# wjmaddox/online_gp

Hardware: AMD Instinct MI355X
Metric: streaming updates/sec (WISKI, 50^3 inducing grid) (higher is better)
Workload: dtype f32

## Files before the change

include/wiski.h:

```cpp
#ifndef WISKI_H
#define WISKI_H

#include <stdint.h>

#ifdef __cplusplus
extern "C" {
#endif

#define WISKI_OK 0
#define WISKI_E_BADARG (-1)
#define WISKI_E_LAUNCH (-2)
#define WISKI_E_WORKSPACE (-3)
#define WISKI_E_NOTCONV (-4)
#define WISKI_PENDING 1

#define WISKI_MAX_DIM 4

typedef struct wiski_grid {
  int32_t d;
  int32_t g[WISKI_MAX_DIM];
  double g0[WISKI_MAX_DIM];
  double h[WISKI_MAX_DIM];
} wiski_grid;

// ... 99 lines not shown
  int32_t guard_ok;
  double shift;
} wiski_pcg_async;
int wiski_pcg_async_f32(const wiski_grid* grid, const float* d_A_st, const float* d_tcol, float kscale, const float* d_evec, const float* d_evec2, const float* d_eval, float shift, const float* d_RHS, int32_t k, float* d_U, float* d_Z, int32_t warm, double tol, int32_t max_iter, int32_t check_every, int32_t first_check, void* d_work, int64_t work_bytes, int32_t* h_iters, double* h_relres, const int32_t* d_err, int32_t* h_err, int32_t a_sym, float* d_R, void* stream, wiski_pcg_async* handle, int32_t mode);
int wiski_pcg_async_f64(const wiski_grid* grid, const double* d_A_st, const double* d_tcol, double kscale, const double* d_evec, const double* d_evec2, const double* d_eval, double shift, const double* d_RHS, int32_t k, double* d_U, double* d_Z, int32_t warm, double tol, int32_t max_iter, int32_t check_every, int32_t first_check, void* d_work, int64_t work_bytes, int32_t* h_iters, double* h_relres, const int32_t* d_err, int32_t* h_err, int32_t a_sym, double* d_R, void* stream, wiski_pcg_async* handle, int32_t mode);
int wiski_pcg_async_free(wiski_pcg_async* handle);
int wiski_pcg_async_guard(const wiski_pcg_async* handle, const void** d_guard, int64_t* expect);
int wiski_pcg_zero_regions_f32(const wiski_grid* grid, int32_t k, int32_t max_iter, void* d_work, int32_t a_sym, void** p1, int64_t* n1_bytes, void** p2, int64_t* n2_bytes);
int wiski_pcg_zero_regions_f64(const wiski_grid* grid, int32_t k, int32_t max_iter, void* d_work, int32_t a_sym, void** p1, int64_t* n1_bytes, void** p2, int64_t* n2_bytes);
int64_t wiski_scatter_bin_bytes(const wiski_grid* grid, int64_t n, int32_t elem_size);
int wiski_scatter_stats_step_f32(const wiski_grid* grid, const float* d_x, const float* d_y, const float* d_wa, const float* d_wb, const float* d_noise, int64_t n, float* d_b, float* d_A_half, float* d_cnt, const float* d_u, float* d_res, float* d_mean_out, double* d_stats, int32_t* d_err, void* z1, int64_t n1_bytes, void* z2, int64_t n2_bytes, const void* d_guard, int64_t guard_expect, void* d_bin, int64_t bin_bytes, void* stream);
int wiski_scatter_stats_step_f64(const wiski_grid* grid, const double* d_x, const double* d_y, const double* d_wa, const double* d_wb, const double* d_noise, int64_t n, double* d_b, double* d_A_half, double* d_cnt, const double* d_u, double* d_res, double* d_mean_out, double* d_stats, int32_t* d_err, void* z1, int64_t n1_bytes, void* z2, int64_t n2_bytes, const void* d_guard, int64_t guard_expect, void* d_bin, int64_t bin_bytes, void* stream);
int wiski_gather_zero_f32(const wiski_grid* grid, const float* d_x, int64_t n, const float* d_V, int32_t k, float* d_out, int32_t* d_err, void* z1, int64_t n1_bytes, void* z2, int64_t n2_bytes, int32_t* zeroed, void* stream);
int wiski_gather_zero_f64(const wiski_grid* grid, const double* d_x, int64_t n, const double* d_V, int32_t k, double* d_out, int32_t* d_err, void* z1, int64_t n1_bytes, void* z2, int64_t n2_bytes, int32_t* zeroed, void* stream);

typedef struct wiski_stream_args_f32 {
  float* d_A_half; float* d_b; float* d_cnt; double* d_stats; int32_t* d_err;
  float* d_U; float* d_Z; float* d_R;
  const float* d_tcol; float kscale; const float* d_evec; const float* d_evec2; const float* d_eval; float shift;
  double tol; int32_t max_iter; int32_t check_every; void* d_work; int64_t work_bytes;
  void* d_bin; int64_t bin_bytes;
  const wiski_shard* shard;
  const wiski_twolevel* two_level;
  int32_t keep[3];
} wiski_stream_args_f32;
typedef struct wiski_stream_args_f64 {
  double* d_A_half; double* d_b; double* d_cnt; double* d_stats; int32_t* d_err;
  double* d_U; double* d_Z; double* d_R;
  const double* d_tcol; double kscale; const double* d_evec; const double* d_evec2; const double* d_eval; double shift;
  double tol; int32_t max_iter; int32_t check_every; void* d_work; int64_t work_bytes;
  void* d_bin; int64_t bin_bytes;
  const wiski_shard* shard;
  const wiski_twolevel* two_level;
  int32_t keep[3];
} wiski_stream_args_f64;
int wiski_stream_step_f32(const wiski_grid* grid, const wiski_stream_args_f32* args, const float* d_x, const float* d_y, const float* d_wa, const float* d_wb, const float* d_noise, int64_t q, float* d_mean_out, int32_t carry, int32_t first_check, int32_t* h_iters, double* h_relres, int32_t* h_err, void* stream, wiski_pcg_async* handle, int32_t defer, int32_t* h_resumed);
int wiski_stream_step_f64(const wiski_grid* grid, const wiski_stream_args_f64* args, const double* d_x, const double* d_y, const double* d_wa, const double* d_wb, const double* d_noise, int64_t q, double* d_mean_out, int32_t carry, int32_t first_check, int32_t* h_iters, double* h_relres, int32_t* h_err, void* stream, wiski_pcg_async* handle, int32_t defer, int32_t* h_resumed);

int wiski_scatter_stats_multi_f32(const wiski_grid* grid, const float* d_x, const float* d_y, const float* d_wa, const float* d_wb, const float* d_noise, int64_t n, int32_t nout, int64_t y_stride, int64_t w_stride, float* d_b, float* d_A_half, int64_t A_stride, float* d_cnt, const float* d_u, float* d_res, double* d_stats, int32_t* d_err, void* stream);
int wiski_scatter_stats_multi_f64(const wiski_grid* grid, const double* d_x, const double* d_y, const double* d_wa, const double* d_wb, const double* d_noise, int64_t n, int32_t nout, int64_t y_stride, int64_t w_stride, double* d_b, double* d_A_half, int64_t A_stride, double* d_cnt, const double* d_u, double* d_res, double* d_stats, int32_t* d_err, void* stream);

int wiski_scatter_stats_grad_f32(const wiski_grid* grid, const float* d_x, const float* d_y, const float* d_wa, const float* d_wb, const float* d_noise, int64_t n, float* d_b, float* d_A_half, float* d_cnt, const float* d_u, float* d_res, float* d_mean_out, double* d_stats, int32_t* d_err, void* stream);
int wiski_scatter_stats_grad_f64(const wiski_grid* grid, const double* d_x, const double* d_y, const double* d_wa, const double* d_wb, const double* d_noise, int64_t n, double* d_b, double* d_A_half, double* d_cnt, const double* d_u, double* d_res, double* d_mean_out, double* d_stats, int32_t* d_err, void* stream);

typedef struct wiski_absorb_args {
  const void* d_x; const void* d_y; const void* d_wa; const void* d_wb; const void* d_noise; int64_t n;
  void* d_b; void* d_A; int32_t half; int32_t channels; void* d_cnt; double* d_stats; int32_t* d_err;
  const void* d_u; void* d_res; void* d_mean_out;
  void* z1; int64_t n1_bytes; void* z2; int64_t n2_bytes;
  const void* d_guard; int64_t guard_expect;
  void* d_bin; int64_t bin_bytes;
  int32_t g_lo; int32_t g_hi; int32_t nout; int32_t reserved;
  int64_t y_stride; int64_t w_stride; int64_t A_stride;
} wiski_absorb_args;
int wiski_absorb_f32(const wiski_grid* grid, const wiski_absorb_args* args, void* stream);
int wiski_absorb_f64(const wiski_grid* grid, const wiski_absorb_args* args, void* stream);

int wiski_scatter_stats_robust_f32(const wiski_grid* grid, const float* d_x, const float* d_y, const float* d_wa, const float* d_wb, const float* d_noise, int64_t n, float* d_b, float* d_A_half, float* d_cnt, const float* d_u, float* d_res, float* d_mean_out, double* d_stats, int32_t* d_err, const float* d_inv_scale, float huber_c, float* d_omega_out, void* stream);
int wiski_scatter_stats_robust_f64(const wiski_grid* grid, const double* d_x, const double* d_y, const double* d_wa, const double* d_wb, const double* d_noise, int64_t n, double* d_b, double* d_A_half, double* d_cnt, const double* d_u, double* d_res, double* d_mean_out, double* d_stats, int32_t* d_err, const double* d_inv_scale, double huber_c, double* d_omega_out, void* stream);
int wiski_absorb_robust_f32(const wiski_grid* grid, const wiski_absorb_args* args, const float* d_inv_scale, float huber_c, float* d_omega_out, void* stream);
int wiski_absorb_robust_f64(const wiski_grid* grid, const wiski_absorb_args* args, const double* d_inv_scale, double huber_c, double* d_omega_out, void* stream);

typedef struct wiski_window_ring {
  void* d_x; void* d_y; void* d_wa; void* d_wb; void* d_noise;
  int64_t cap; int64_t head;
} wiski_window_ring;
int wiski_scatter_stats_window_f32(const wiski_grid* grid, const float* d_x, const float* d_y, const float* d_wa, const float* d_wb, const float* d_noise, int64_t n, const wiski_window_ring* ring, float* d_b, float* d_A_half, float* d_cnt, const float* d_u, float* d_res, float* d_mean_out, double* d_stats, int32_t* d_err, int32_t* d_void_left, void* stream);
int wiski_scatter_stats_window_f64(const wiski_grid* grid, const double* d_x, const double* d_y, const double* d_wa, const double* d_wb, const double* d_noise, int64_t n, const wiski_window_ring* ring, double* d_b, double* d_A_half, double* d_cnt, const double* d_u, double* d_res, double* d_mean_out, double* d_stats, int32_t* d_err, int32_t* d_void_left, void* stream);
int wiski_absorb_window_f32(const wiski_grid* grid, const wiski_absorb_args* args, const wiski_window_ring* ring, int32_t* d_void_left, void* stream);
int wiski_absorb_window_f64(const wiski_grid* grid, const wiski_absorb_args* args, const wiski_window_ring* ring, int32_t* d_void_left, void* stream);

int wiski_scatter_stats_interval_f32(const wiski_grid* grid, const float* d_x, const float* d_lo, const float* d_hi, const float* d_pvar, double sigma2, const float* d_wa, const float* d_wb, const float* d_noise, int64_t n, float* d_b, float* d_A_half, float* d_cnt, const float* d_u, float* d_res, float* d_mean_out, double* d_stats, int32_t* d_err, float* d_ytilde_out, float* d_omega_out, double* d_logz_out, void* stream);
int wiski_scatter_stats_interval_f64(const wiski_grid* grid, const double* d_x, const double* d_lo, const double* d_hi, const double* d_pvar, double sigma2, const double* d_wa, const double* d_wb, const double* d_noise, int64_t n, double* d_b, double* d_A_half, double* d_cnt, const double* d_u, double* d_res, double* d_mean_out, double* d_stats, int32_t* d_err, double* d_ytilde_out, double* d_omega_out, double* d_logz_out, void* stream);
int wiski_absorb_interval_f32(const wiski_grid* grid, const wiski_absorb_args* args, const float* d_lo, const float* d_hi, const float* d_pvar, double sigma2, float* d_ytilde_out, float* d_omega_out, double* d_logz_out, void* stream);
int wiski_absorb_interval_f64(const wiski_grid* grid, const wiski_absorb_args* args, const double* d_lo, const double* d_hi, const double* d_pvar, double sigma2, double* d_ytilde_out, double* d_omega_out, double* d_logz_out, void* stream);

int wiski_scatter_stats_step_sharded_f32(const wiski_grid* grid, const float* d_x, const float* d_y, const float* d_wa, const float* d_wb, const float* d_noise, int64_t n, float* d_b, float* d_A_half, float* d_cnt, const float* d_u, float* d_res, float* d_mean_out, double* d_stats, int32_t* d_err, void* z1, int64_t n1_bytes, void* z2, int64_t n2_bytes, const void* d_guard, int64_t guard_expect, int32_t g_lo, int32_t g_hi, void* stream);
int wiski_scatter_stats_step_sharded_f64(const wiski_grid* grid, const double* d_x, const double* d_y, const double* d_wa, const double* d_wb, const double* d_noise, int64_t n, double* d_b, double* d_A_half, double* d_cnt, const double* d_u, double* d_res, double* d_mean_out, double* d_stats, int32_t* d_err, void* z1, int64_t n1_bytes, void* z2, int64_t n2_bytes, const void* d_guard, int64_t guard_expect, int32_t g_lo, int32_t g_hi, void* stream);
int wiski_pcg_sharded_f32(const wiski_grid* grid, const float* d_A_st, const float* d_tcol, float kscale, const float* d_evec, const float* d_evec2, const float* d_eval, float shift, const float* d_RHS, int32_t k, float* d_U, float* d_Z, int32_t warm, double tol, int32_t max_iter, int32_t check_every, int32_t first_check, void* d_work, int64_t work_bytes, int32_t* h_iters, double* h_relres, const int32_t* d_err, int32_t* h_err, int32_t a_sym, float* d_R, void* stream, wiski_pcg_async* handle, int32_t mode, const wiski_shard* shard);
int wiski_pcg_sharded_f64(const wiski_grid* grid, const double* d_A_st, const double* d_tcol, double kscale, const double* d_evec, const double* d_evec2, const double* d_eval, double shift, const double* d_RHS, int32_t k, double* d_U, double* d_Z, int32_t warm, double tol, int32_t max_iter, int32_t check_every, int32_t first_check, void* d_work, int64_t work_bytes, int32_t* h_iters, double* h_relres, const int32_t* d_err, int32_t* h_err, int32_t a_sym, double* d_R, void* stream, wiski_pcg_async* handle, int32_t mode, const wiski_shard* shard);
int wiski_pcg_twolevel_f32(const wiski_grid* grid, const float* d_A_st, const float* d_tcol, float kscale, const float* d_evec, const float* d_evec2, const float* d_eval, float shift, const float* d_RHS, int32_t k, float* d_U, float* d_Z, int32_t warm, double tol, int32_t max_iter, int32_t check_every, int32_t first_check, void* d_work, int64_t work_bytes, int32_t* h_iters, double* h_relres, const int32_t* d_err, int32_t* h_err, int32_t a_sym, float* d_R, void* stream, wiski_pcg_async* handle, int32_t mode, const wiski_shard* shard, const wiski_twolevel* two_level);
int64_t wiski_twolevel_refresh_workspace_bytes(int32_t r);
int wiski_twolevel_refresh_f32(const wiski_grid* grid, const float* d_x, int64_t n, const float* d_scale, const double* d_V, int32_t kw, const int32_t* d_S, int32_t r, const double* d_lam_unit, double kscale, double gscale, double* d_G, void* d_work, int64_t work_bytes, float* d_N, const uint64_t* d_sticky, int32_t* d_bad, void* stream);
int wiski_precond_apply_f32(const wiski_grid* grid, const float* d_evec, const float* d_evec2, const float* d_eval, float kscale, float shift, const float* d_r, float* d_w0, float* d_w1, float* d_y, float* d_t, double* d_rho, const wiski_twolevel* two_level, void* stream);
int wiski_precond_apply_keep_f32(const wiski_grid* grid, const float* d_evec, const float* d_evec2, const float* d_eval, float kscale, float shift, const float* d_r, float* d_w0, float* d_w1, float* d_y, float* d_t, double* d_rho, const wiski_twolevel* two_level, const int32_t* keep, void* stream);
int wiski_precond_keep_ok(const wiski_grid* grid, const int32_t* keep, int32_t with_two_level);
int wiski_precond_apply_cols_f32(const wiski_grid* grid, const float* d_evec, const float* d_evec2, const float* d_eval, float kscale, float shift, const float* d_r, int32_t k, float* d_w0, float* d_w1, float* d_y, float* d_t, double* d_rho, const wiski_twolevel* two_level, void* stream);

int wiski_gemm_f32(int32_t ta, int32_t tb, int32_t M, int32_t N, int32_t K, float alpha, const float* d_A, int32_t lda, const float* d_B, int32_t ldb, float beta, float* d_C, int32_t ldc, void* stream);
int wiski_gemm_f64(int32_t ta, int32_t tb, int32_t M, int32_t N, int32_t K, double alpha, const double* d_A, int32_t lda, const double* d_B, int32_t ldb, double beta, double* d_C, int32_t ldc, void* stream);
int wiski_potrf_f32(int32_t n, float* d_A, int32_t lda, int32_t* d_info, void* stream);
int wiski_potrf_f64(int32_t n, double* d_A, int32_t lda, int32_t* d_info, void* stream);
int wiski_potrf_inverse_f32(int32_t n, float* d_A, int32_t lda, float* d_X, int32_t ldx, int32_t* d_info, void* stream);
int wiski_potrf_inverse_f64(int32_t n, double* d_A, int32_t lda, double* d_X, int32_t ldx, int32_t* d_info, void* stream);
int wiski_trsm_f32(int32_t trans, int32_t n, int32_t nrhs, const float* d_L, int32_t ldl, float* d_B, int32_t ldb, void* stream);
int wiski_trsm_f64(int32_t trans, int32_t n, int32_t nrhs, const double* d_L, int32_t ldl, double* d_B, int32_t ldb, void* stream);
int wiski_logdiag_f32(int32_t n, const float* d_A, int32_t lda, double* d_out, void* stream);
int wiski_logdiag_f64(int32_t n, const double* d_A, int32_t lda, double* d_out, void* stream);

int wiski_dense_factor_f32(const wiski_grid* grid, const float* d_A_half, const float* d_evec, const float* d_eval, float kscale, float* d_work, int64_t work_elems, float* d_chol, float* d_M, double* d_logdiag, int32_t* d_info, void* stream);
int wiski_dense_factor_f64(const wiski_grid* grid, const double* d_A_half, const double* d_evec, const double* d_eval, double kscale, double* d_work, int64_t work_elems, double* d_chol, double* d_M, double* d_logdiag, int32_t* d_info, void* stream);

int64_t wiski_root_update_workspace_elems(int32_t m, int32_t r, int32_t q);
int wiski_root_update_f32(int32_t m, int32_t r, int32_t q, float* d_L, int32_t ldl, float* d_R, int32_t ldr, const float* d_V, int32_t ldv, float* d_ws, int64_t ws_elems, void* stream);
int wiski_root_update_f64(int32_t m, int32_t r, int32_t q, double* d_L, int32_t ldl, double* d_R, int32_t ldr, const double* d_V, int32_t ldv, double* d_ws, int64_t ws_elems, void* stream);

int wiski_basis_project_f32(const wiski_grid* grid, const float* d_x, int64_t n, const double* d_V, int32_t kmax, const int32_t* d_S, int32_t r, const float* d_scale, const double* d_colscale, const double* d_tcol, double* d_F, int64_t ldf, double* d_prior, int32_t* d_err, void* stream);
int wiski_basis_project_f64(const wiski_grid* grid, const double* d_x, int64_t n, const double* d_V, int32_t kmax, const int32_t* d_S, int32_t r, const double* d_scale, const double* d_colscale, const double* d_tcol, double* d_F, int64_t ldf, double* d_prior, int32_t* d_err, void* stream);
int wiski_basis_project_vjp_f32(const wiski_grid* grid, const float* d_x, int64_t n, const double* d_V, int32_t kmax, const int32_t* d_S, int32_t r, const float* d_scale, const double* d_colscale, const double* d_tcol, const double* d_GF, int64_t ldg, const double* d_Gprior, float* d_gx, void* stream);
int wiski_basis_project_vjp_f64(const wiski_grid* grid, const double* d_x, int64_t n, const double* d_V, int32_t kmax, const int32_t* d_S, int32_t r, const double* d_scale, const double* d_colscale, const double* d_tcol, const double* d_GF, int64_t ldg, const double* d_Gprior, double* d_gx, void* stream);
int wiski_basis_absorb_h_f32(int64_t n, int32_t r, const double* d_F, int64_t ldf, const float* d_wby, const float* d_scale, double* d_h, void* stream);
int wiski_basis_absorb_h_f64(int64_t n, int32_t r, const double* d_F, int64_t ldf, const double* d_wby, const double* d_scale, double* d_h, void* stream);
int wiski_factor_refresh_layout(int32_t d, int64_t nV, int32_t kw, int32_t r_ref, int32_t r, int64_t* off);
int wiski_factor_refresh(int32_t d, const int32_t* d_g, int64_t nV, const double* d_tcol, const double* d_Vin, int32_t kw, int32_t kuse, const double* d_Vref, int32_t kref, int32_t niter, double resid_ok, const int32_t* d_Sref, const int32_t* d_S, int32_t r_ref, int32_t r, double* d_work, double* d_verdict, const double* d_Gref, const double* d_href, double kscale, int32_t* d_info, double* d_out, void* verdict_event, void* stream);
int wiski_basis_pair_reduce(int32_t d, int32_t r, int32_t kmax, const double* d_Wt, const int32_t* d_S, const double* d_ev, double* d_D, void* stream);
int wiski_basis_eig_update(int32_t d, const int32_t* d_g, const double* d_tcol, const double* d_Vin, int32_t kw, int32_t kuse, double* d_Vout, double* d_ev, double* d_resid,
                           const double* d_Vref, int32_t kref, double* d_Tq, void* stream);
int wiski_basis_eig_update_adaptive(int32_t d, const int32_t* d_g, const double* d_tcol, const double* d_Vin, int32_t kw, int32_t kuse, double* d_Vout, double* d_ev, double* d_resid, const double* d_Vref, int32_t kref, double* d_Tq, int32_t niter, double resid_ok, void* stream);
int wiski_basis_change(int32_t d, const int32_t* d_g, int32_t kref, int32_t kw, int32_t r_ref, int32_t r, const double* d_Tq, const int32_t* d_Sref, const int32_t* d_S, const double* d_ev, const double* d_tcol, const double* d_resid, double* d_TS, double* d_lam, double* d_work, double* d_verdict, void* stream);
int wiski_basis_lag_grad(int32_t d, const int32_t* d_g, int32_t kw, const double* d_V, const double* d_D, double scale, const double* d_scale, double* d_out, void* stream);
int wiski_spectral_var(int32_t n, int32_t r, const double* d_Y, const double* d_F, const double* d_prior, double kscale, double* d_diag, double* d_tail, void* stream);
#define WISKI_HYPER_MAX_PARAMS 6
typedef struct {
  void* raw;
  void* exp_avg;
  void* exp_avg_sq;
  void* step;
  int32_t numel;
  int32_t step_numel;
  int32_t role;
  int32_t kind;
  double lower, upper;
} wiski_hyper_param;
typedef struct {
  int32_t count;
  int32_t reserved;
  wiski_hyper_param p[WISKI_HYPER_MAX_PARAMS];
} wiski_hyper_plan;
int wiski_hyper_columns_f32(const wiski_hyper_plan* plan, const wiski_grid* grid, int32_t kind, float* d_ell, float* d_scale, float* d_s2, double* d_s2_f64, double* d_tcol64, float* d_tcol, void* stream);
int wiski_hyper_columns_f64(const wiski_hyper_plan* plan, const wiski_grid* grid, int32_t kind, double* d_ell, double* d_scale, double* d_s2, double* d_s2_f64, double* d_tcol64, double* d_tcol, void* stream);
int wiski_hyper_mid_f32(const double* d_bMb, const double* d_logdet, const float* d_s2, const double* d_c, const double* d_ld, const double* d_n, double* d_out, double* d_loss, void* stream);
int wiski_hyper_mid_f64(const double* d_bMb, const double* d_logdet, const double* d_s2, const double* d_c, const double* d_ld, const double* d_n, double* d_out, double* d_loss, void* stream);
int wiski_hyper_adam_f32(const wiski_hyper_plan* plan, const float* d_scale, const float* d_s2, const float* d_gell, const float* d_gscale, const double* d_mid, const double* d_gkap, const double* d_n, double lr, double beta1, double beta2, double eps, void* stream);
int wiski_hyper_adam_f64(const wiski_hyper_plan* plan, const double* d_scale, const double* d_s2, const double* d_gell, const double* d_gscale, const double* d_mid, const double* d_gkap, const double* d_n, double lr, double beta1, double beta2, double eps, void* stream);
#define WISKI_COPY_MAX_SEGMENTS 12
typedef struct {
  const void* src[WISKI_COPY_MAX_SEGMENTS];
  void* dst[WISKI_COPY_MAX_SEGMENTS];
  int64_t n[WISKI_COPY_MAX_SEGMENTS];
  int32_t count;
  int32_t reserved;
  double scalar;
  void* scalar_dst;
} wiski_copy_plan;
int wiski_multi_copy_f64(const wiski_copy_plan* plan, void* stream);
int wiski_spectral_evaluate_f32(int32_t n, int32_t r, const double* d_F, const double* d_prior, const double* d_Linv, int32_t ldl, const double* d_t, double kscale, const float* d_s2, const float* d_y, const int32_t* d_err, double* d_ws, double* d_out, float* d_mean, float* d_var, void* stream);
int wiski_spectral_evaluate_f64(int32_t n, int32_t r, const double* d_F, const double* d_prior, const double* d_Linv, int32_t ldl, const double* d_t, double kscale, const double* d_s2, const double* d_y, const int32_t* d_err, double* d_ws, double* d_out, double* d_mean, double* d_var, void* stream);
int wiski_spectral_evaluate_y_f32(int32_t n, int32_t r, const double* d_Y, const double* d_F, const double* d_prior, const double* d_t, double kscale, const float* d_s2, const float* d_y, const int32_t* d_err, double* d_ws, double* d_out, float* d_mean, float* d_var, void* stream);
int wiski_spectral_evaluate_y_f64(int32_t n, int32_t r, const double* d_Y, const double* d_F, const double* d_prior, const double* d_t, double kscale, const double* d_s2, const double* d_y, const int32_t* d_err, double* d_ws, double* d_out, double* d_mean, double* d_var, void* stream);
int wiski_factor_tail(int32_t r_ref, int32_t r, const double* d_TS, const double* d_href, const double* d_sq, const double* d_Linv, const double* d_chol, double* d_out, void* stream);
int wiski_woodbury_c(int32_t r, const double* d_G, const double* d_lam_kuu, double kscale, double* d_C, double* d_lam, double* d_sq, double* d_sqG, void* stream);
int wiski_mll_weights(int32_t r, const double* d_G, const double* d_P, const double* d_zeta, const double* d_lam_kuu, const double* d_gb, const double* d_gld, double* d_Wt, double* d_gkap, void* stream);

int wiski_comm_unique_id_bytes(void);
int wiski_comm_unique_id(void* id_out);
int wiski_comm_init_rank(const void* id_bytes, int32_t nranks, int32_t rank, void** comm_out);
// ... 58 lines not shown
```

online_gp_amd/csrc/two_level.hip:

```cpp
#include "wiski_common.h"

extern "C" void wiski_potrf_quiet(int on);

using tl_f64x4 = __attribute__((ext_vector_type(4))) double;

__global__ __launch_bounds__(256) void k_gram_acc(int n, int r, int chunk, const double* __restrict__ F, int64_t ldf, double* __restrict__ G) {
  __shared__ double sA[32][33];
  __shared__ double sB[32][33];
  const int tid = threadIdx.x, lane = tid & 63, w = tid >> 6;
  const int qa = w >> 1, qb = w & 1;
  int ti = (int)((sqrtf(8.f * (float)blockIdx.x + 1.f) - 1.f) * 0.5f);
  while ((ti + 1) * (ti + 2) / 2 <= (int)blockIdx.x) ++ti;
  while (ti * (ti + 1) / 2 > (int)blockIdx.x) --ti;
  const int tj = (int)blockIdx.x - ti * (ti + 1) / 2;
  const int i0 = ti * 32, j0 = tj * 32;
  const int p_lo = blockIdx.y * chunk;
  const int p_hi = min(n, p_lo + chunk);
  const int r8 = tid >> 3, c4 = (tid & 7) * 4;
  tl_f64x4 acc = {0.0, 0.0, 0.0, 0.0};
  double pa[4], pb[4];
  auto fetch = [&](int p0) {
    const int p = p0 + r8;
#pragma unroll
    for (int u = 0; u < 4; ++u) {
      const int gi = i0 + c4 + u, gj = j0 + c4 + u;
      pa[u] = (p < p_hi && gi < r) ? F[(int64_t)p * ldf + gi] : 0.0;
      pb[u] = (p < p_hi && gj < r) ? F[(int64_t)p * ldf + gj] : 0.0;
    }
  };
  fetch(p_lo);
  for (int p0 = p_lo; p0 < p_hi; p0 += 32) {
#pragma unroll
    for (int u = 0; u < 4; ++u) {
      sA[r8][c4 + u] = pa[u];
      sB[r8][c4 + u] = pb[u];
    }
    __syncthreads();
    if (p0 + 32 < p_hi) fetch(p0 + 32);
#pragma unroll
    for (int ks = 0; ks < 32; ks += 4) {
      const int kk = ks + (lane >> 4);
      acc = __builtin_amdgcn_mfma_f64_16x16x4f64(sA[kk][qa * 16 + (lane & 15)], sB[kk][qb * 16 + (lane & 15)], acc, 0, 0, 0);
    }
    __syncthreads();
  }
#pragma unroll
  for (int q = 0; q < 4; ++q) {
    const int gi = i0 + qa * 16 + (lane >> 4) + 4 * q, gj = j0 + qb * 16 + (lane & 15);
    if (gi < r && gj < r) {
      unsafeAtomicAdd(G + (int64_t)gi * r + gj, acc[q]);
      if (ti != tj) unsafeAtomicAdd(G + (int64_t)gj * r + gi, acc[q]);
    }
  }
}

__global__ void k_tl_scale_cast(int r, const double* __restrict__ T, const double* __restrict__ sq, double inv_gscale, const int32_t* __restrict__ info,
                                float* __restrict__ N, const unsigned long long* __restrict__ sticky, int32_t* bad) {
  const int e = blockIdx.x * blockDim.x + threadIdx.x;
  if (e < r * r) {
    const int i = e / r, j = e - i * r;
    const float v = *info ? __builtin_nanf("") : (float)(sq[i] * sq[j] * T[e] * inv_gscale);
    N[e] = v;
    if (bad) {
      int b = (e == 0 && *info) || !(fabsf(v) <= 3.4028234e38f) ? 1 : 0;
      if (e == 0 && sticky && *sticky != 0ull) b |= 2;
      if (b) __hip_atomic_fetch_or(bad, b, __ATOMIC_RELAXED, __HIP_MEMORY_SCOPE_SYSTEM);
    }
  }
}

constexpr int TL_CHUNK_POINTS = 16384;

static inline int64_t tl_align(int64_t v) { return (v + 255) & ~(int64_t)255; }

extern "C" {
int64_t wiski_twolevel_refresh_workspace_bytes(int32_t r) {
  if (r < 1 || r > 512) return WISKI_E_BADARG;
  return tl_align((int64_t)TL_CHUNK_POINTS * r * 8) + 3 * tl_align((int64_t)r * r * 8) + 2 * tl_align((int64_t)r * 8) + tl_align(16);
}

int wiski_twolevel_refresh_f32(const wiski_grid* grid, const float* d_x, int64_t n, const float* d_scale, const double* d_V, int32_t kw, const int32_t* d_S,
                               int32_t r, const double* d_lam_unit, double kscale, double gscale, double* d_G, void* d_work, int64_t work_bytes, float* d_N,
                               const uint64_t* d_sticky, int32_t* d_bad,
                               void* stream) {
  if (!(gscale > 0)) return WISKI_E_BADARG;
  if (!grid || n < 0 || (n > 0 && !d_x) || !d_V || !d_S || r < 1 || r > 512 || !d_lam_unit || !d_G || !d_work || !d_N) return WISKI_E_BADARG;
  if (work_bytes < wiski_twolevel_refresh_workspace_bytes(r)) return WISKI_E_WORKSPACE;
  hipStream_t s = (hipStream_t)stream;
  char* w = (char*)d_work;
  double* F = (double*)w;                 w += tl_align((int64_t)TL_CHUNK_POINTS * r * 8);
  double* C = (double*)w;                 w += tl_align((int64_t)r * r * 8);
  double* Li = (double*)w;                w += tl_align((int64_t)r * r * 8);
  double* T = (double*)w;                 w += tl_align((int64_t)r * r * 8);
  double* lam = (double*)w;               w += tl_align((int64_t)r * 8);
  double* sq = (double*)w;                w += tl_align((int64_t)r * 8);
  const int nt32 = (r + 31) / 32, nt = nt32 * (nt32 + 1) / 2;
  int32_t* info = (int32_t*)w;
  for (int64_t p0 = 0; p0 < n; p0 += TL_CHUNK_POINTS) {
    const int64_t nc = n - p0 < TL_CHUNK_POINTS ? n - p0 : TL_CHUNK_POINTS;
    if (int rc = wiski_basis_project_f32(grid, d_x + p0 * grid->d, nc, d_V, kw, d_S, r, d_scale ? d_scale + p0 : nullptr, nullptr, nullptr, F, r, nullptr,
                                         nullptr, stream))
      return rc;
    int chunk = (int)((nc * nt + 383) / 384);
    chunk = (chunk + 31) & ~31;
    if (chunk < 256) chunk = 256;
    const int ny = (int)((nc + chunk - 1) / chunk);
    hipLaunchKernelGGL(k_gram_acc, dim3((unsigned)nt, (unsigned)ny), dim3(256), 0, s, (int)nc, (int)r, chunk, (const double*)F, (int64_t)r, d_G);
    if (hipGetLastError() != hipSuccess) return WISKI_E_LAUNCH;
  }
  if (int rc = wiski_woodbury_c(r, d_G, d_lam_unit, kscale * gscale, C, lam, sq, nullptr, stream)) return rc;
  if (hipMemsetAsync(info, 0, sizeof(int32_t), s) != hipSuccess) return WISKI_E_LAUNCH;
  {
    static const bool quiet = [] { const char* e = getenv("WISKI_TL_QUIET_POTRF"); return !(e && e[0] == '0'); }();
    if (quiet) wiski_potrf_quiet(1);
    const int rcp = wiski_potrf_inverse_f64(r, C, r, Li, r, info, stream);
    if (quiet) wiski_potrf_quiet(0);
    if (rcp) return rcp;
  }
  if (int rc = wiski_gemm_f64(1, 0, r, r, r, 1.0, Li, r, Li, r, 0.0, T, r, stream)) return rc;
  hipLaunchKernelGGL(k_tl_scale_cast, dim3((unsigned)((r * r + 255) / 256)), dim3(256), 0, s, (int)r, (const double*)T, (const double*)sq, 1.0 / gscale,
                     (const int32_t*)info, d_N, (const unsigned long long*)d_sticky, d_bad);
  return hipGetLastError() == hipSuccess ? WISKI_OK : WISKI_E_LAUNCH;
}
}
```

online_gp_amd/lazy/two_level.py:

```python
import ctypes

import numpy as np
import torch

from .. import _hip, grid_ops, settings

_SIDE = {}
_WORK = {}
KMAX = 32
MC_COLS = 64
MAXR = 480


def select_modes(D_host, kscale, rank):
    d = len(D_host)
    tops = [np.arange(len(D))[::-1][:KMAX] for D in D_host]
    lam = D_host[0][tops[0]]
    for q in range(1, d):
        lam = np.multiply.outer(lam, D_host[q][tops[q]])
    flat = lam.reshape(-1)
    r = int(min(rank, flat.size, MAXR))
    sel = np.argsort(-flat, kind="stable")[:r]
    sub = np.stack(np.unravel_index(sel, lam.shape))
    idx = np.stack([tops[q][sub[q]] for q in range(d)])
    order = np.lexsort(tuple(idx[q] for q in range(d - 1, -1, -1)))
    idx = idx[:, order]
    lam_sel = flat[sel][order] * kscale
    return idx.astype(np.int64), lam_sel


class TwoLevelBlock:

    def __init__(self, grid, device, eig_host, kscale, rank, err):
        assert grid.d == 3 and max(grid.g) <= 64
        self.grid, self.device, self.err = grid, device, err
        X, D = eig_host["X"], eig_host["D"]
        idx, lam = select_modes(D, kscale, rank)
        self.r = r = idx.shape[1]
        self.idx_host = idx
        g0 = grid.g[0]
        off = np.zeros(g0 + 1, dtype=np.int32)
        np.add.at(off[1:], idx[0], 1)
        off = np.cumsum(off).astype(np.int32)
        mask = np.zeros((g0, 64), dtype=np.uint64)
        for j in range(r):
            mask[idx[0, j], idx[1, j]] |= np.uint64(1) << np.uint64(idx[2, j])
        pos = (idx[1] * 256 + idx[2]).astype(np.uint16)
        self.nslab = int((np.diff(off) > 0).sum())
        self.d_off = torch.as_tensor(off).to(device)
        self.d_mask = torch.as_tensor(mask.view(np.int64).reshape(-1)).to(device)
        self.d_pos = torch.as_tensor(pos.view(np.int16)).to(device)
        self.d_cs = torch.zeros(max(r, 4) + 1, dtype=torch.int64, device=device)
        self.N = [torch.zeros((r, r), dtype=torch.float32, device=device) for _ in range(2)]
        self.active = -1
        self.mc = torch.empty((2, MC_COLS, r), dtype=torch.float32, device=device)
        self.struct = grid_ops.TwoLevelStruct(r, self.nslab, self.d_mask.data_ptr(), self.d_off.data_ptr(), self.d_pos.data_ptr(),
                                              self.N[0].data_ptr(), self.d_cs.data_ptr(), self.mc.data_ptr(), MC_COLS)
        kw = int(max((len(D[q]) - 1 - idx[q]).max() for q in range(3))) + 1
        self.kw = kw
        tabs = [np.ascontiguousarray(X[q][:, ::-1][:, :kw]) for q in range(3)]
        self.Vtab = torch.as_tensor(np.concatenate([t.reshape(-1) for t in tabs])).to(device)
        S = np.stack([len(D[q]) - 1 - idx[q] for q in range(3)]).astype(np.int32)
        self.S = torch.as_tensor(S).to(device).contiguous()
        self._S_long = self.S.long()
        self.lam_unit = torch.as_tensor(lam / kscale).to(device)
        self.kscale = float(kscale)
        self.G = torch.zeros((r, r), dtype=torch.float64, device=device)
        wkey = (str(device), r)
        if wkey not in _WORK:
            nb = int(_hip.lib().wiski_twolevel_refresh_workspace_bytes(ctypes.c_int32(r)))
            _WORK[wkey] = torch.empty(nb, dtype=torch.uint8, device=device)
        self.work = _WORK[wkey]
        if str(device) not in _SIDE:
            side = None
            h = ctypes.c_void_p()
            with torch.cuda.device(device):
                if _hip.lib().wiski_side_stream_create(ctypes.c_int32(1), ctypes.byref(h)) == 0 and h.value:
                    side = torch.cuda.ExternalStream(h.value, device=device)
            _SIDE[str(device)] = side if side is not None else torch.cuda.Stream(device=device)
        self.side = _SIDE[str(device)]
        self.in_flight = None
        self.failed = False
        self.weight_at_launch = 0.0
        self.refreshes = 0

    def ensure_cols(self, k):
        if k > self.struct.mc_cols:
            self.mc = torch.empty((2, int(k), self.r), dtype=torch.float32, device=self.device)
            self.struct.d_mc, self.struct.mc_cols = self.mc.data_ptr(), int(k)

    def launch_refresh(self, points, step, weight, gscale=1.0, subsample=None):
        tgt = 1 - self.active if self.active >= 0 else 0
        if len(points) == 1:
            X, wa = points[0]
        else:
            X = torch.cat([p_[0] for p_ in points], dim=0)
            wa = None if all(p_[1] is None for p_ in points) else torch.cat(
                [p_[1] if p_[1] is not None else torch.ones(p_[0].shape[0], dtype=p_[0].dtype, device=self.device) for p_ in points])
        sc = None if wa is None else wa.to(X.dtype).sqrt().contiguous()
        sub = subsample if subsample else settings.two_level_subsample.value()
        if sub > 1 and X.shape[0] >= 64 * sub:
            X = X[::sub]
            sc = (sc[::sub] * (sub ** 0.5)).contiguous() if sc is not None else torch.full((X.shape[0],), float(sub) ** 0.5, dtype=X.dtype, device=self.device)
        X = X.contiguous()
        main = torch.cuda.current_stream(self.device)
        ready = torch.cuda.Event()
        ready.record(main)
        with torch.cuda.stream(self.side):
            self.side.wait_event(ready)
            X.record_stream(self.side)
            if sc is not None:
                sc.record_stream(self.side)
            X = X.contiguous()
            if getattr(self, "_bad_host", None) is None:
                self._bad_host = torch.zeros(1, dtype=torch.int32).pin_memory()
            self._bad_host[0] = 0
            rc = _hip.lib().wiski_twolevel_refresh_f32(self.grid.ref, _hip.dptr(X), ctypes.c_int64(X.shape[0]), _hip.dptr(sc), _hip.dptr(self.Vtab),
                                                        ctypes.c_int32(self.kw), _hip.dptr(self.S), ctypes.c_int32(self.r), _hip.dptr(self.lam_unit),
                                                        ctypes.c_double(self.kscale), ctypes.c_double(gscale), _hip.dptr(self.G), _hip.dptr(self.work),
                                                        ctypes.c_int64(self.work.numel()), _hip.dptr(self.N[tgt]),
                                                        ctypes.c_void_p(self.d_cs.data_ptr() + 8 * self.r), ctypes.c_void_p(self._bad_host.data_ptr()),
                                                        _hip.stream_ptr(self.device))
            _hip.check(rc, "wiski_twolevel_refresh")
            self._keep = (X, sc)
            done = torch.cuda.Event()
            done.record(self.side)
        self.in_flight = (done, step, tgt)
        self.weight_at_launch = weight
        self.refreshes += 1

    def rebase(self, eig_host, kscale):
        X, D = eig_host["X"], eig_host["D"]
        idx = self.idx_host
        lam = np.ones(self.r)
        for q in range(3):
            lam = lam * D[q][idx[q]]
        tabs = [np.ascontiguousarray(X[q][:, ::-1][:, :self.kw]) for q in range(3)]
        self.Vtab.copy_(torch.as_tensor(np.concatenate([t.reshape(-1) for t in tabs])))
        self.lam_unit.copy_(torch.as_tensor(lam))
        self.kscale = float(kscale)
        self.active, self.in_flight, self.failed = -1, None, False
        self.rebases = getattr(self, "rebases", 0) + 1

    def rebuild_from_stencil(self, stencil, weight):
        g, dev, r = self.grid.g, self.device, self.r
        torch.cuda.current_stream(dev).wait_stream(self.side)
        Vq, o = [], 0
        for q in range(3):
            Vq.append(self.Vtab[o:o + g[q] * self.kw].reshape(g[q], self.kw).float())
            o += g[q] * self.kw
        S = self._S_long
        step = r if r * self.grid.m * 4 <= (1 << 28) else 64
        G = torch.empty((r, r), dtype=torch.float32, device=dev)
        for lo in range(0, r, step):
            hi = min(lo + step, r)
            c = hi - lo
            Bc = Vq[0][:, S[0, lo:hi]].t()
            for q in (1, 2):
                Bc = Bc.reshape(c, -1, 1) * Vq[q][:, S[q, lo:hi]].t().reshape(c, 1, -1)
            AB = grid_ops.stencil_spmv(self.grid, stencil, Bc.reshape(c, self.grid.m).contiguous())
            P = AB.reshape((c,) + tuple(g))
            for q in range(3):
                P = torch.tensordot(P, Vq[q], dims=([1], [0]))
            G[lo:hi] = P[(slice(None), S[0], S[1], S[2])]
        G = G.double()
        self.G = (0.5 * (G + G.t())).contiguous()
        if getattr(self, "_bad_host", None) is None:
            self._bad_host = torch.zeros(1, dtype=torch.int32).pin_memory()
        self._bad_host[0] = 0
        rc = _hip.lib().wiski_twolevel_refresh_f32(self.grid.ref, None, ctypes.c_int64(0), None, _hip.dptr(self.Vtab), ctypes.c_int32(self.kw),
                                                    _hip.dptr(self.S), ctypes.c_int32(r), _hip.dptr(self.lam_unit), ctypes.c_double(self.kscale),
                                                    ctypes.c_double(1.0), _hip.dptr(self.G), _hip.dptr(self.work), ctypes.c_int64(self.work.numel()),
                                                    _hip.dptr(self.N[0]), ctypes.c_void_p(self.d_cs.data_ptr() + 8 * self.r),
                                                    ctypes.c_void_p(self._bad_host.data_ptr()), _hip.stream_ptr(dev))
        _hip.check(rc, "wiski_twolevel_refresh")
        done = torch.cuda.Event()
        done.record(torch.cuda.current_stream(dev))
        done.synchronize()
        if int(self._bad_host[0]):
            self.failed = True
            self.active = -1
            return False
        self.active = 0
        self.struct.d_N = self.N[0].data_ptr()
        self.in_flight = None
        self.weight_at_launch = weight
        self.refreshes += 1
        self.rebuilt = True
        return True

    def tick(self, step, lag, lockstep=False):
        fl = self.in_flight
        if fl is None:
            return False
        done, at, tgt = fl
        if lockstep:
            if step < at + lag:
                return False
            done.synchronize()
        elif not done.query():
            if step < at + 4 * max(lag, 1):
                return False
            done.synchronize()
        self.in_flight = None
        if int(self._bad_host[0]):
            self.failed = True
            return False
        self.active = tgt
        self.struct.d_N = self.N[tgt].data_ptr()
        return True

    def finish(self):
        if self.in_flight is not None:
            self.tick(self.in_flight[1] + 10 ** 9, 0, lockstep=True)


class TwoLevelTracker:

    def __init__(self):
        self.pending = []
        self.pending_n = 0
        self.covered = True
        self.block = None
        self.block_key = None
        self.step = 0
        self.switched = False
        self.seen_iters = []
        self.last_q = 0
        self.wanted = False
        self.rebuilds = 0

    def reset(self):
        self.__init__()

    def note(self, X, wa):
        if not self.covered:
            return
        self.pending.append((X, wa))
        self.pending_n += X.shape[0]
        if self.block is None and self.pending_n > 4_000_000:
            self.lose()

    def lose(self):
        if self.block is not None and not self.block.failed:
            self._spare = self.block
        self.pending, self.pending_n, self.covered, self.block, self.block_key = [], 0, False, None, None

    def rebuild(self, grid, device, pst, kscale, stencil, weight, err):
        if not self.wanted or pst is None or "eig_host" not in pst or settings.two_level_rebuild.off():
            return None
        blk = getattr(self, "_spare", None)
        self._spare = None
        if (blk is not None and blk.grid is grid and blk.r == min(settings.two_level_rank.value(), MAXR) and getattr(blk, "rebases", 0) % 32 != 31
                and (blk.in_flight is None or blk.in_flight[0].query())):
            blk.rebase(pst["eig_host"], kscale)
        else:
            blk = TwoLevelBlock(grid, device, pst["eig_host"], kscale, settings.two_level_rank.value(), err)
        if not blk.rebuild_from_stencil(stencil, weight):
            self.rebuild_failures = getattr(self, "rebuild_failures", 0) + 1
            return None
        self.block, self.block_key, self._eig_ref = blk, (id(pst["eig"][0]), float(kscale), settings.two_level_rank.value()), pst["eig"]
        self.pending, self.pending_n, self.covered = [], 0, True
        self.rebuilds += 1
        return blk.struct

    def current(self, pst, kscale, cols=1):
        blk = self.block
        if (blk is None or not self.covered or blk.failed or blk.active < 0 or pst is None or "eig" not in pst or
                self.block_key != (id(pst["eig"][0]), float(kscale), settings.two_level_rank.value())):
            return None
        blk.ensure_cols(cols)
        return blk.struct

    def for_step(self, grid, device, pst, kscale, weight, err, lockstep=False, last_iters=0, subsample=None):
        if not self.covered or "eig_host" not in pst:
            return None
        key = (id(pst["eig"][0]), float(kscale), settings.two_level_rank.value())
        if self.block is None or self.block_key != key:
            if self.block is not None:
                self.lose()
                return None
            if last_iters > 0:
                self.seen_iters.append(last_iters)
            if len(self.seen_iters) < 3:
                return None
            if min(self.seen_iters[1:3]) < settings.two_level_min_iters.value():
                if len(self.seen_iters) >= 6:
                    self.lose()
# ... 21 lines not shown
```

Baseline: 26.03 million.

## Gather two-level refresh batches on device instead of torch cat and subsample

Adds a batched refresh entry point. A pack kernel on the side stream gathers and subsamples points directly from each batch's pointers and computes the sqrt-weight scale. This replaces the host-side torch.cat, slicing, sqrt and stream/event management, which launched several small kernels and allocated intermediate tensors. The pinned verdict flag is also read through a ctypes word instead of tensor indexing. The cost is an extra pack kernel per chunk, host-side slice loops, and a global in-flight list that keeps input tensors alive until their refresh completes.

After: 25.66 million. 0.986x the previous value.

```diff
diff --git a/include/wiski.h b/include/wiski.h
--- a/include/wiski.h
+++ b/include/wiski.h
@@ -205,6 +205,7 @@
 int wiski_pcg_twolevel_f32(const wiski_grid* grid, const float* d_A_st, const float* d_tcol, float kscale, const float* d_evec, const float* d_evec2, const float* d_eval, float shift, const float* d_RHS, int32_t k, float* d_U, float* d_Z, int32_t warm, double tol, int32_t max_iter, int32_t check_every, int32_t first_check, void* d_work, int64_t work_bytes, int32_t* h_iters, double* h_relres, const int32_t* d_err, int32_t* h_err, int32_t a_sym, float* d_R, void* stream, wiski_pcg_async* handle, int32_t mode, const wiski_shard* shard, const wiski_twolevel* two_level);
 int64_t wiski_twolevel_refresh_workspace_bytes(int32_t r);
 int wiski_twolevel_refresh_f32(const wiski_grid* grid, const float* d_x, int64_t n, const float* d_scale, const double* d_V, int32_t kw, const int32_t* d_S, int32_t r, const double* d_lam_unit, double kscale, double gscale, double* d_G, void* d_work, int64_t work_bytes, float* d_N, const uint64_t* d_sticky, int32_t* d_bad, void* stream);
+int wiski_twolevel_refresh_batches_f32(const wiski_grid* grid, const float* const* h_x, const int64_t* h_n, const float* const* h_wa, int32_t nb, int32_t sub, const double* d_V, int32_t kw, const int32_t* d_S, int32_t r, const double* d_lam_unit, double kscale, double gscale, double* d_G, void* d_work, int64_t work_bytes, float* d_N, const uint64_t* d_sticky, int32_t* d_bad, void* main_stream, void* side_stream);
 int wiski_precond_apply_f32(const wiski_grid* grid, const float* d_evec, const float* d_evec2, const float* d_eval, float kscale, float shift, const float* d_r, float* d_w0, float* d_w1, float* d_y, float* d_t, double* d_rho, const wiski_twolevel* two_level, void* stream);
 int wiski_precond_apply_keep_f32(const wiski_grid* grid, const float* d_evec, const float* d_evec2, const float* d_eval, float kscale, float shift, const float* d_r, float* d_w0, float* d_w1, float* d_y, float* d_t, double* d_rho, const wiski_twolevel* two_level, const int32_t* keep, void* stream);
 int wiski_precond_keep_ok(const wiski_grid* grid, const int32_t* keep, int32_t with_two_level);
diff --git a/online_gp_amd/csrc/two_level.hip b/online_gp_amd/csrc/two_level.hip
--- a/online_gp_amd/csrc/two_level.hip
+++ b/online_gp_amd/csrc/two_level.hip
@@ -1,4 +1,5 @@
 #include "wiski_common.h"
+#include <mutex>
 
 extern "C" void wiski_potrf_quiet(int on);
 
@@ -70,13 +71,107 @@
 }
 
 constexpr int TL_CHUNK_POINTS = 16384;
+constexpr int TL_SLICE = 64;
 
 static inline int64_t tl_align(int64_t v) { return (v + 255) & ~(int64_t)255; }
+
+struct tl_batch_slice {
+  const float* x[TL_SLICE];
+  const float* wa[TL_SLICE];
+  int64_t start[TL_SLICE + 1];
+  int32_t nb;
+};
+
+__global__ __launch_bounds__(256) void k_tl_pack(const tl_batch_slice t, int d, int64_t k0, int nc, int sub, float sqrt_sub, float* __restrict__ xo,
+                                                 float* __restrict__ so) {
+  const int k = blockIdx.x * blockDim.x + threadIdx.x;
+  if (k >= nc) return;
+  const int64_t c = (k0 + k) * (int64_t)sub;
+  if (c < t.start[0] || c >= t.start[t.nb]) return;
+  int lo = 0, hi = t.nb;
+  while (hi - lo > 1) {
+    const int mid = (lo + hi) >> 1;
+    if (t.start[mid] <= c) lo = mid; else hi = mid;
+  }
+  const int64_t p = c - t.start[lo];
+  const float* __restrict__ xs = t.x[lo] + p * d;
+  for (int q = 0; q < d; ++q) xo[(int64_t)k * d + q] = xs[q];
+  const float* wa = t.wa[lo];
+  so[k] = (wa ? sqrtf(wa[p]) : 1.f) * sqrt_sub;
+}
+
+struct tl_work {
+  double *F, *C, *Li, *T, *lam, *sq;
+  int32_t* info;
+  float *px, *ps;
+};
+
+static tl_work tl_carve(void* d_work, int r) {
+  tl_work k;
+  char* w = (char*)d_work;
+  k.F = (double*)w;                       w += tl_align((int64_t)TL_CHUNK_POINTS * r * 8);
+  k.C = (double*)w;                       w += tl_align((int64_t)r * r * 8);
+  k.Li = (double*)w;                      w += tl_align((int64_t)r * r * 8);
+  k.T = (double*)w;                       w += tl_align((int64_t)r * r * 8);
+  k.lam = (double*)w;                     w += tl_align((int64_t)r * 8);
+  k.sq = (double*)w;                      w += tl_align((int64_t)r * 8);
+  k.info = (int32_t*)w;                   w += tl_align(16);
+  k.px = (float*)w;                       w += tl_align((int64_t)TL_CHUNK_POINTS * WISKI_MAX_DIM * 4);
+  k.ps = (float*)w;
+  return k;
+}
+
+static int tl_accumulate(const wiski_grid* grid, const float* d_x, int64_t nc, const float* d_scale, const double* d_V, int32_t kw, const int32_t* d_S, int32_t r,
+                         double* F, double* d_G, void* stream) {
+  const int nt32 = (r + 31) / 32, nt = nt32 * (nt32 + 1) / 2;
+  if (int rc = wiski_basis_project_f32(grid, d_x, nc, d_V, kw, d_S, r, d_scale, nullptr, nullptr, F, r, nullptr, nullptr, stream)) return rc;
+  int chunk = (int)((nc * nt + 383) / 384);
+  chunk = (chunk + 31) & ~31;
+  if (chunk < 256) chunk = 256;
+  const int ny = (int)((nc + chunk - 1) / chunk);
+  hipLaunchKernelGGL(k_gram_acc, dim3((unsigned)nt, (unsigned)ny), dim3(256), 0, (hipStream_t)stream, (int)nc, (int)r, chunk, (const double*)F, (int64_t)r, d_G);
+  return hipGetLastError() == hipSuccess ? WISKI_OK : WISKI_E_LAUNCH;
+}
+
+static int tl_factor(const tl_work& k, int32_t r, const double* d_lam_unit, double kscale, double gscale, const double* d_G, float* d_N, const uint64_t* d_sticky,
+                     int32_t* d_bad, void* stream) {
+  hipStream_t s = (hipStream_t)stream;
+  if (int rc = wiski_woodbury_c(r, d_G, d_lam_unit, kscale * gscale, k.C, k.lam, k.sq, nullptr, stream)) return rc;
+  if (hipMemsetAsync(k.info, 0, sizeof(int32_t), s) != hipSuccess) return WISKI_E_LAUNCH;
+  {
+    static const bool quiet = [] { const char* e = getenv("WISKI_TL_QUIET_POTRF"); return !(e && e[0] == '0'); }();
+    if (quiet) wiski_potrf_quiet(1);
+    const int rcp = wiski_potrf_inverse_f64(r, k.C, r, k.Li, r, k.info, stream);
+    if (quiet) wiski_potrf_quiet(0);
+    if (rcp) return rcp;
+  }
+  if (int rc = wiski_gemm_f64(1, 0, r, r, r, 1.0, k.Li, r, k.Li, r, 0.0, k.T, r, stream)) return rc;
+  hipLaunchKernelGGL(k_tl_scale_cast, dim3((unsigned)((r * r + 255) / 256)), dim3(256), 0, s, (int)r, (const double*)k.T, (const double*)k.sq, 1.0 / gscale,
+                     (const int32_t*)k.info, d_N, (const unsigned long long*)d_sticky, d_bad);
+  return hipGetLastError() == hipSuccess ? WISKI_OK : WISKI_E_LAUNCH;
+}
+
+static int tl_side_after_main(hipStream_t main, hipStream_t side) {
+  constexpr int MAXDEV = 64;
+  static hipEvent_t ev[MAXDEV];
+  static bool have[MAXDEV];
+  static std::mutex mu;
+  int dev = 0;
+  if (hipGetDevice(&dev) != hipSuccess || dev < 0 || dev >= MAXDEV) return WISKI_E_LAUNCH;
+  std::lock_guard<std::mutex> lock(mu);
+  if (!have[dev]) {
+    if (hipEventCreateWithFlags(&ev[dev], hipEventDisableTiming) != hipSuccess) return WISKI_E_LAUNCH;
+    have[dev] = true;
+  }
+  if (hipEventRecord(ev[dev], main) != hipSuccess || hipStreamWaitEvent(side, ev[dev], 0) != hipSuccess) return WISKI_E_LAUNCH;
+  return WISKI_OK;
+}
 
 extern "C" {
 int64_t wiski_twolevel_refresh_workspace_bytes(int32_t r) {
   if (r < 1 || r > 512) return WISKI_E_BADARG;
-  return tl_align((int64_t)TL_CHUNK_POINTS * r * 8) + 3 * tl_align((int64_t)r * r * 8) + 2 * tl_align((int64_t)r * 8) + tl_align(16);
+  return tl_align((int64_t)TL_CHUNK_POINTS * r * 8) + 3 * tl_align((int64_t)r * r * 8) + 2 * tl_align((int64_t)r * 8) + tl_align(16) +
+         tl_align((int64_t)TL_CHUNK_POINTS * WISKI_MAX_DIM * 4) + tl_align((int64_t)TL_CHUNK_POINTS * 4);
 }
 
 int wiski_twolevel_refresh_f32(const wiski_grid* grid, const float* d_x, int64_t n, const float* d_scale, const double* d_V, int32_t kw, const int32_t* d_S,
@@ -86,40 +181,59 @@
   if (!(gscale > 0)) return WISKI_E_BADARG;
   if (!grid || n < 0 || (n > 0 && !d_x) || !d_V || !d_S || r < 1 || r > 512 || !d_lam_unit || !d_G || !d_work || !d_N) return WISKI_E_BADARG;
   if (work_bytes < wiski_twolevel_refresh_workspace_bytes(r)) return WISKI_E_WORKSPACE;
-  hipStream_t s = (hipStream_t)stream;
-  char* w = (char*)d_work;
-  double* F = (double*)w;                 w += tl_align((int64_t)TL_CHUNK_POINTS * r * 8);
-  double* C = (double*)w;                 w += tl_align((int64_t)r * r * 8);
-  double* Li = (double*)w;                w += tl_align((int64_t)r * r * 8);
-  double* T = (double*)w;                 w += tl_align((int64_t)r * r * 8);
-  double* lam = (double*)w;               w += tl_align((int64_t)r * 8);
-  double* sq = (double*)w;                w += tl_align((int64_t)r * 8);
-  const int nt32 = (r + 31) / 32, nt = nt32 * (nt32 + 1) / 2;
-  int32_t* info = (int32_t*)w;
+  const tl_work k = tl_carve(d_work, r);
   for (int64_t p0 = 0; p0 < n; p0 += TL_CHUNK_POINTS) {
     const int64_t nc = n - p0 < TL_CHUNK_POINTS ? n - p0 : TL_CHUNK_POINTS;
-    if (int rc = wiski_basis_project_f32(grid, d_x + p0 * grid->d, nc, d_V, kw, d_S, r, d_scale ? d_scale + p0 : nullptr, nullptr, nullptr, F, r, nullptr,
-                                         nullptr, stream))
-      return rc;
-    int chunk = (int)((nc * nt + 383) / 384);
-    chunk = (chunk + 31) & ~31;
-    if (chunk < 256) chunk = 256;
-    const int ny = (int)((nc + chunk - 1) / chunk);
-    hipLaunchKernelGGL(k_gram_acc, dim3((unsigned)nt, (unsigned)ny), dim3(256), 0, s, (int)nc, (int)r, chunk, (const double*)F, (int64_t)r, d_G);
-    if (hipGetLastError() != hipSuccess) return WISKI_E_LAUNCH;
-  }
-  if (int rc = wiski_woodbury_c(r, d_G, d_lam_unit, kscale * gscale, C, lam, sq, nullptr, stream)) return rc;
-  if (hipMemsetAsync(info, 0, sizeof(int32_t), s) != hipSuccess) return WISKI_E_LAUNCH;
-  {
-    static const bool quiet = [] { const char* e = getenv("WISKI_TL_QUIET_POTRF"); return !(e && e[0] == '0'); }();
-    if (quiet) wiski_potrf_quiet(1);
-    const int rcp = wiski_potrf_inverse_f64(r, C, r, Li, r, info, stream);
-    if (quiet) wiski_potrf_quiet(0);
-    if (rcp) return rcp;
-  }
-  if (int rc = wiski_gemm_f64(1, 0, r, r, r, 1.0, Li, r, Li, r, 0.0, T, r, stream)) return rc;
-  hipLaunchKernelGGL(k_tl_scale_cast, dim3((unsigned)((r * r + 255) / 256)), dim3(256), 0, s, (int)r, (const double*)T, (const double*)sq, 1.0 / gscale,
-                     (const int32_t*)info, d_N, (const unsigned long long*)d_sticky, d_bad);
-  return hipGetLastError() == hipSuccess ? WISKI_OK : WISKI_E_LAUNCH;
-}
-}
+    if (int rc = tl_accumulate(grid, d_x + p0 * grid->d, nc, d_scale ? d_scale + p0 : nullptr, d_V, kw, d_S, r, k.F, d_G, stream)) return rc;
+  }
+  return tl_factor(k, r, d_lam_unit, kscale, gscale, d_G, d_N, d_sticky, d_bad, stream);
+}
+
+int wiski_twolevel_refresh_batches_f32(const wiski_grid* grid, const float* const* h_x, const int64_t* h_n, const float* const* h_wa, int32_t nb, int32_t sub,
+                                       const double* d_V, int32_t kw, const int32_t* d_S, int32_t r, const double* d_lam_unit, double kscale, double gscale,
+                                       double* d_G, void* d_work, int64_t work_bytes, float* d_N, const uint64_t* d_sticky, int32_t* d_bad, void* main_stream,
+                                       void* side_stream) {
+  if (!(gscale > 0)) return WISKI_E_BADARG;
+  if (!grid || grid->d < 1 || grid->d > WISKI_MAX_DIM || !h_x || !h_n || nb < 1 || sub < 1 || !d_V || !d_S || r < 1 || r > 512 || !d_lam_unit || !d_G ||
+      !d_work || !d_N)
+    return WISKI_E_BADARG;
+  int64_t total = 0;
+  for (int32_t b = 0; b < nb; ++b) {
+    if (h_n[b] < 0 || (h_n[b] > 0 && !h_x[b])) return WISKI_E_BADARG;
+    total += h_n[b];
+  }
+  if (work_bytes < wiski_twolevel_refresh_workspace_bytes(r)) return WISKI_E_WORKSPACE;
+  hipStream_t side = (hipStream_t)side_stream;
+  if (int rc = tl_side_after_main((hipStream_t)main_stream, side)) return rc;
+  const tl_work k = tl_carve(d_work, r);
+  const int d = grid->d;
+  const float sqrt_sub = (float)sqrt((double)sub);
+  const int64_t nsel = (total + sub - 1) / sub;
+  int32_t b_lo = 0;
+  int64_t s_lo = 0;
+  for (int64_t k0 = 0; k0 < nsel; k0 += TL_CHUNK_POINTS) {
+    const int nc = (int)(nsel - k0 < TL_CHUNK_POINTS ? nsel - k0 : TL_CHUNK_POINTS);
+    const int64_t c_first = k0 * sub, c_last = (k0 + nc - 1) * sub;
+    while (s_lo + h_n[b_lo] <= c_first) s_lo += h_n[b_lo++];
+    int32_t b = b_lo;
+    int64_t s = s_lo;
+    while (b < nb && s <= c_last) {
+      tl_batch_slice t;
+      t.nb = nb - b < TL_SLICE ? nb - b : TL_SLICE;
+      for (int32_t i = 0; i < TL_SLICE; ++i) {
+        const bool in = i < t.nb;
+        t.x[i] = in ? h_x[b + i] : nullptr;
+        t.wa[i] = in && h_wa ? h_wa[b + i] : nullptr;
+        t.start[i] = s;
+        if (in) s += h_n[b + i];
+      }
+      t.start[TL_SLICE] = s;
+      b += t.nb;
+      hipLaunchKernelGGL(k_tl_pack, dim3((unsigned)((nc + 255) / 256)), dim3(256), 0, side, t, d, k0, nc, (int)sub, sqrt_sub, k.px, k.ps);
+      if (hipGetLastError() != hipSuccess) return WISKI_E_LAUNCH;
+    }
+    if (int rc = tl_accumulate(grid, k.px, nc, k.ps, d_V, kw, d_S, r, k.F, d_G, side_stream)) return rc;
+  }
+  return tl_factor(k, r, d_lam_unit, kscale, gscale, d_G, d_N, d_sticky, d_bad, side_stream);
+}
+}
diff --git a/online_gp_amd/lazy/two_level.py b/online_gp_amd/lazy/two_level.py
--- a/online_gp_amd/lazy/two_level.py
+++ b/online_gp_amd/lazy/two_level.py
@@ -9,6 +9,7 @@
 _WORK = {}
 KMAX = 32
 MC_COLS = 64
+_INFLIGHT = []
 MAXR = 480
 
 
@@ -89,42 +90,45 @@
             self.mc = torch.empty((2, int(k), self.r), dtype=torch.float32, device=self.device)
             self.struct.d_mc, self.struct.mc_cols = self.mc.data_ptr(), int(k)
 
+    def _verdict_word(self):
+        if getattr(self, "_bad_host", None) is None:
+            self._bad_host = torch.zeros(1, dtype=torch.int32).pin_memory()
+            self._bad_word = ctypes.c_int32.from_address(self._bad_host.data_ptr())
+        return self._bad_word
+
     def launch_refresh(self, points, step, weight, gscale=1.0, subsample=None):
         tgt = 1 - self.active if self.active >= 0 else 0
-        if len(points) == 1:
-            X, wa = points[0]
-        else:
-            X = torch.cat([p_[0] for p_ in points], dim=0)
-            wa = None if all(p_[1] is None for p_ in points) else torch.cat(
-                [p_[1] if p_[1] is not None else torch.ones(p_[0].shape[0], dtype=p_[0].dtype, device=self.device) for p_ in points])
-        sc = None if wa is None else wa.to(X.dtype).sqrt().contiguous()
+        nb = len(points)
+        xs, ns, was = (ctypes.c_void_p * nb)(), (ctypes.c_int64 * nb)(), (ctypes.c_void_p * nb)()
+        keep, total = [], 0
+        for b, (X, wa) in enumerate(points):
+            if X.dtype != torch.float32 or not X.is_contiguous():
+                X = X.to(torch.float32).contiguous()
+            xs[b], ns[b] = X.data_ptr(), X.shape[0]
+            total += X.shape[0]
+            keep.append(X)
+            if wa is not None:
+                if wa.dtype != torch.float32 or not wa.is_contiguous():
+                    wa = wa.to(torch.float32).contiguous()
+                was[b] = wa.data_ptr()
+                keep.append(wa)
         sub = subsample if subsample else settings.two_level_subsample.value()
-        if sub > 1 and X.shape[0] >= 64 * sub:
-            X = X[::sub]
-            sc = (sc[::sub] * (sub ** 0.5)).contiguous() if sc is not None else torch.full((X.shape[0],), float(sub) ** 0.5, dtype=X.dtype, device=self.device)
-        X = X.contiguous()
-        main = torch.cuda.current_stream(self.device)
-        ready = torch.cuda.Event()
-        ready.record(main)
-        with torch.cuda.stream(self.side):
-            self.side.wait_event(ready)
-            X.record_stream(self.side)
-            if sc is not None:
-                sc.record_stream(self.side)
-            X = X.contiguous()
-            if getattr(self, "_bad_host", None) is None:
-                self._bad_host = torch.zeros(1, dtype=torch.int32).pin_memory()
-            self._bad_host[0] = 0
-            rc = _hip.lib().wiski_twolevel_refresh_f32(self.grid.ref, _hip.dptr(X), ctypes.c_int64(X.shape[0]), _hip.dptr(sc), _hip.dptr(self.Vtab),
-                                                        ctypes.c_int32(self.kw), _hip.dptr(self.S), ctypes.c_int32(self.r), _hip.dptr(self.lam_unit),
-                                                        ctypes.c_double(self.kscale), ctypes.c_double(gscale), _hip.dptr(self.G), _hip.dptr(self.work),
-                                                        ctypes.c_int64(self.work.numel()), _hip.dptr(self.N[tgt]),
-                                                        ctypes.c_void_p(self.d_cs.data_ptr() + 8 * self.r), ctypes.c_void_p(self._bad_host.data_ptr()),
-                                                        _hip.stream_ptr(self.device))
-            _hip.check(rc, "wiski_twolevel_refresh")
-            self._keep = (X, sc)
-            done = torch.cuda.Event()
-            done.record(self.side)
+        if not (sub > 1 and total >= 64 * sub):
+            sub = 1
+        bad = self._verdict_word()
+        bad.value = 0
+        rc = _hip.lib().wiski_twolevel_refresh_batches_f32(self.grid.ref, xs, ns, was, ctypes.c_int32(nb), ctypes.c_int32(int(sub)), _hip.dptr(self.Vtab),
+                                                            ctypes.c_int32(self.kw), _hip.dptr(self.S), ctypes.c_int32(self.r), _hip.dptr(self.lam_unit),
+                                                            ctypes.c_double(self.kscale), ctypes.c_double(gscale), _hip.dptr(self.G), _hip.dptr(self.work),
+                                                            ctypes.c_int64(self.work.numel()), _hip.dptr(self.N[tgt]),
+                                                            ctypes.c_void_p(self.d_cs.data_ptr() + 8 * self.r), ctypes.c_void_p(self._bad_host.data_ptr()),
+                                                            _hip.stream_ptr(self.device), ctypes.c_void_p(self.side.cuda_stream))
+        _hip.check(rc, "wiski_twolevel_refresh_batches")
+        done = torch.cuda.Event()
+        done.record(self.side)
+        self._keep = keep
+        _INFLIGHT[:] = [e for e in _INFLIGHT if not e[0].query()]
+        _INFLIGHT.append((done, keep))
         self.in_flight = (done, step, tgt)
         self.weight_at_launch = weight
         self.refreshes += 1
@@ -165,9 +169,7 @@
             G[lo:hi] = P[(slice(None), S[0], S[1], S[2])]
         G = G.double()
         self.G = (0.5 * (G + G.t())).contiguous()
-        if getattr(self, "_bad_host", None) is None:
-            self._bad_host = torch.zeros(1, dtype=torch.int32).pin_memory()
-        self._bad_host[0] = 0
+        self._verdict_word().value = 0
         rc = _hip.lib().wiski_twolevel_refresh_f32(self.grid.ref, None, ctypes.c_int64(0), None, _hip.dptr(self.Vtab), ctypes.c_int32(self.kw),
                                                     _hip.dptr(self.S), ctypes.c_int32(r), _hip.dptr(self.lam_unit), ctypes.c_double(self.kscale),
                                                     ctypes.c_double(1.0), _hip.dptr(self.G), _hip.dptr(self.work), ctypes.c_int64(self.work.numel()),
@@ -177,7 +179,7 @@
         done = torch.cuda.Event()
         done.record(torch.cuda.current_stream(dev))
         done.synchronize()
-        if int(self._bad_host[0]):
+        if self._bad_word.value:
             self.failed = True
             self.active = -1
             return False
@@ -203,7 +205,7 @@
                 return False
             done.synchronize()
         self.in_flight = None
-        if int(self._bad_host[0]):
+        if self._bad_word.value:
             self.failed = True
             return False
         self.active = tgt
```
